# csxmli2016/MARCONet

Hardware: NVIDIA H100
Metric: sr_chars_per_sec (higher is better)
Workload: dtype f32

## Files before the change

marconet_b200/csrc/conv_small.cu:

```cuda
#include "conv_common.cuh"
#include "mn_common.cuh"

namespace {

constexpr int PH = 8, PW = 32, CCH = 16;
constexpr int PIX_PITCH = CCH + 4;

template <int COUT>
__global__ void __launch_bounds__(PH * PW) conv3x3_small_cout_kernel(const ConvGeom g) {
    mn_pdl_prologue();
    __shared__ __align__(16) float halo[(PH + 2) * (PW + 2) * PIX_PITCH];
    __shared__ __align__(16) float wsm[9 * CCH * 4];
    const int tx = threadIdx.x % PW, ty = threadIdx.x / PW;
    const int tiles_w = (g.W + PW - 1) / PW, tiles_h = (g.H + PH - 1) / PH;
    int b = blockIdx.x;
    const int twi = b % tiles_w; b /= tiles_w;
    const int thi = b % tiles_h;
    const int n = b / tiles_h;
    const int ox0 = twi * PW, oy0 = thi * PH;
    const float* xn = g.x + (size_t)n * g.H * g.W * g.x_cs;
    float acc[4] = {0.f, 0.f, 0.f, 0.f};
    for (int c0 = 0; c0 < g.Cin; c0 += CCH) {
        __syncthreads();
        for (int i = threadIdx.x; i < (PH + 2) * (PW + 2) * (CCH / 4); i += PH * PW) {
            const int q = i % (CCH / 4), pix = i / (CCH / 4);
            const int hx = pix % (PW + 2), hy = pix / (PW + 2);
            const int iy = oy0 + hy - 1, ix = ox0 + hx - 1;
            float4 v = make_float4(0.f, 0.f, 0.f, 0.f);
            if ((unsigned)iy < (unsigned)g.H && (unsigned)ix < (unsigned)g.W)
                v = __ldg(reinterpret_cast<const float4*>(xn + ((size_t)iy * g.W + ix) * g.x_cs + c0 + q * 4));
            *reinterpret_cast<float4*>(&halo[pix * PIX_PITCH + q * 4]) = v;
        }
        for (int i = threadIdx.x; i < 9 * CCH * 4; i += PH * PW) {
            const int o = i & 3, c = (i >> 2) % CCH, tap = i / (4 * CCH);
            wsm[i] = o < COUT ? __ldg(g.w + ((size_t)tap * g.Cin + c0 + c) * g.Cout + o) : 0.f;
        }
        __syncthreads();
#pragma unroll
        for (int ky = 0; ky < 3; ++ky)
#pragma unroll
            for (int kx = 0; kx < 3; ++kx) {
                const float* hp = &halo[((ty + ky) * (PW + 2) + tx + kx) * PIX_PITCH];
                const float* wp = &wsm[(ky * 3 + kx) * CCH * 4];
#pragma unroll
                for (int q = 0; q < CCH / 4; ++q) {
                    const float4 a = *reinterpret_cast<const float4*>(hp + q * 4);
                    const float av[4] = {a.x, a.y, a.z, a.w};
#pragma unroll
                    for (int j = 0; j < 4; ++j) {
                        const float4 wv = *reinterpret_cast<const float4*>(wp + (q * 4 + j) * 4);
                        acc[0] = fmaf(av[j], wv.x, acc[0]);
                        if (COUT > 1) acc[1] = fmaf(av[j], wv.y, acc[1]);
                        if (COUT > 2) acc[2] = fmaf(av[j], wv.z, acc[2]);
                        if (COUT > 3) acc[3] = fmaf(av[j], wv.w, acc[3]);
                    }
                }
            }
    }
    const int oy = oy0 + ty, ox = ox0 + tx;
    if (oy < g.H && ox < g.W) {
        const int m = (n * g.H + oy) * g.W + ox;
        conv_epilogue4(g, m, 0, acc);
    }
}

}

bool mn_conv_small_supported(const ConvGeom& g) {
    return g.KH == 3 && g.KW == 3 && g.sh == 1 && g.sw == 1 && g.ph == 1 && g.pw == 1 && g.Cout <= 4 && g.Cin % 16 == 0 &&
           g.x_cs % 4 == 0 && (reinterpret_cast<uintptr_t>(g.x) & 15) == 0;
}

int mn_conv_small_launch(const ConvGeom& g, cudaStream_t st) {
    const int blocks = g.N * ((g.H + PH - 1) / PH) * ((g.W + PW - 1) / PW);
    switch (g.Cout) {
        case 1: MN_CUDA_CHECK((mn_launch(conv3x3_small_cout_kernel<1>, dim3(blocks), dim3(PH * PW), 0, st, g))); break;
        case 2: MN_CUDA_CHECK((mn_launch(conv3x3_small_cout_kernel<2>, dim3(blocks), dim3(PH * PW), 0, st, g))); break;
        case 3: MN_CUDA_CHECK((mn_launch(conv3x3_small_cout_kernel<3>, dim3(blocks), dim3(PH * PW), 0, st, g))); break;
        default: MN_CUDA_CHECK((mn_launch(conv3x3_small_cout_kernel<4>, dim3(blocks), dim3(PH * PW), 0, st, g))); break;
    }
    MN_LAUNCH_CHECK();
    return MN_OK;
}
```

marconet_b200/csrc/conv_tc2.cu:

```cuda
#include <cuda.h>
#include <cuda_bf16.h>
#include <cuda_fp16.h>

#include "conv_common.cuh"
#include "mn_common.cuh"
#include "tc_ptx.cuh"

namespace {
using namespace tcptx;

constexpr int KB = 64;
constexpr int NUM_THREADS2 = 512;
constexpr int REG_SPLIT = 88, REG_PROD = 24, REG_CONS = 200;
static_assert(REG_SPLIT + REG_PROD + 2 * REG_CONS <= 4 * 128, "register budget");
constexpr int MAX_HS = 3;
constexpr int MAX_BSTAGES = 4;
__host__ __device__ constexpr int b_half(int nt) { return nt * 128; }
__host__ __device__ constexpr int b_stage(int nt) { return 2 * b_half(nt); }
constexpr int STG_PITCH = 72;
constexpr int STG_BYTES = 128 * STG_PITCH * 4;
constexpr int SMEM_LIMIT = 232448;

template <int A> struct ActTag { static constexpr int value = A; };

struct GnAcc {
    float p = 0.f, s = 0.f, q = 0.f;
    int c = 0;
    __device__ __forceinline__ void add(const float4 w) {
        if (c == 0) p = w.x;
        const float d0 = w.x - p, d1 = w.y - p, d2 = w.z - p, d3 = w.w - p;
        s += (d0 + d1) + (d2 + d3);
        q = fmaf(d0, d0, fmaf(d1, d1, fmaf(d2, d2, fmaf(d3, d3, q))));
        c += 4;
    }
    __device__ __forceinline__ void sums(double& sum, double& sq) const {
        const double pd = p, cd = c;
        sum = cd * pd + s;
        sq = (double)q + 2.0 * pd * s + cd * pd * pd;
    }
};

template <bool GN, int MODE, int NT>
__global__ void __launch_bounds__(NUM_THREADS2, 1)
conv_tc2_kernel(const __grid_constant__ CUtensorMap tmA, const __grid_constant__ CUtensorMap tmBhi,
                const __grid_constant__ CUtensorMap tmBlo, const ConvGeom g, const Tc2Geom t) {
    constexpr int B_HALF = b_half(NT), B_STAGE = b_stage(NT);
    extern __shared__ uint8_t smem_raw[];
    uint8_t* smem = smem_raw + ((1024u - (smem_u32(smem_raw) & 1023u)) & 1023u);
    const uint32_t smem_base = smem_u32(smem);
    const int HS = t.hstages;
    const uint32_t off_b = HS * t.halo_stage_bytes;
    const uint32_t off_stg = off_b + t.bstages * B_STAGE;
    const uint32_t off_rowm = off_stg + STG_BYTES;
    const uint32_t off_bars = off_rowm + 1024;
    float* stg = reinterpret_cast<float*>(smem + off_stg);
    int* rowm = reinterpret_cast<int*>(smem + off_rowm);
    uint64_t* bars = reinterpret_cast<uint64_t*>(smem + off_bars);
    constexpr int I_HF = 0, I_HE = MAX_HS, I_SD = 2 * MAX_HS, I_BF = 3 * MAX_HS, I_BE = I_BF + MAX_BSTAGES;
    auto bar = [&](int i) { return smem_u32(bars + i); };

    const int warp = threadIdx.x >> 5, lane = threadIdx.x & 31;
    const int cs = t.cs;
    const uint32_t crank = cs > 1 ? cluster_ctarank() : 0u;
    const uint16_t cmask = (uint16_t)((1u << cs) - 1u);
    const int num_clusters = gridDim.x / cs;
    auto first_work = [&]() { return (int)(blockIdx.x / cs); };
    const int total_work = t.m_groups * t.n_tiles * t.ksplit;
    const int BS = t.bstages;
    const int units = t.per_tap ? t.cbps * t.taps : t.cbps;
    const int unit_taps = t.per_tap ? 1 : t.taps;
    auto work_ks = [&](int work) { return work % t.ksplit; };
    auto work_nt = [&](int work) { return (work / t.ksplit) % t.n_tiles; };
    auto work_mg = [&](int work) { return work / (t.ksplit * t.n_tiles); };

    if (threadIdx.x == 0) {
        asm volatile("prefetch.tensormap [%0];" ::"l"(&tmA) : "memory");
        asm volatile("prefetch.tensormap [%0];" ::"l"(&tmBhi) : "memory");
        asm volatile("prefetch.tensormap [%0];" ::"l"(&tmBlo) : "memory");
        for (int s = 0; s < MAX_HS; ++s) { mbar_init(bar(I_HF + s), 1); mbar_init(bar(I_HE + s), 2); mbar_init(bar(I_SD + s), 128); }
        for (int s = 0; s < MAX_BSTAGES; ++s) { mbar_init(bar(I_BF + s), 1); mbar_init(bar(I_BE + s), 2 * cs); }
        fence_barrier_init();
    }
    __syncthreads();
    if (cs > 1) cluster_sync_all();
    asm volatile("griddepcontrol.wait;" ::: "memory");
    asm volatile("griddepcontrol.launch_dependents;" ::: "memory");

    auto tile_origin = [&](int work, int& n0, int& oy0, int& ox0) {
        int m_tile = work_mg(work) * cs + (int)crank;
        if (m_tile >= t.m_tiles) { n0 = g.N + 1024; oy0 = 0; ox0 = 0; return; }
        const int tw_i = m_tile % t.tiles_w; m_tile /= t.tiles_w;
        const int th_i = m_tile % t.tiles_h; m_tile /= t.tiles_h;
        n0 = m_tile * t.TN; oy0 = th_i * t.TH; ox0 = tw_i * t.TW;
    };

    if (warp >= 4 && warp < 8) {
        setmaxnreg_dec<REG_PROD>();
        if (warp == 4) {
            uint32_t s = 0, ph = 0;
            const int rows = NT / cs;
            const uint32_t dst0 = smem_base + off_b + crank * rows * 128;
            for (int work = first_work(); work < total_work; work += num_clusters) {
                const int row0 = work_nt(work) * NT + (int)crank * rows;
                const int cb0 = work_ks(work) * t.cbps;
                for (int cb = cb0; cb < cb0 + t.cbps; ++cb) {
                    for (int tap = 0; tap < t.taps; ++tap) {
                        mbar_wait(bar(I_BE + s), ph ^ 1);
                        if (elect_one_sync()) {
                            const uint32_t dst = dst0 + s * B_STAGE;
                            mbar_expect_tx(bar(I_BF + s), B_STAGE);
                            if (cs > 1) {
                                tma_load_3d_mc(&tmBhi, bar(I_BF + s), dst, cb * KB, row0, tap, cmask);
                                tma_load_3d_mc(&tmBlo, bar(I_BF + s), dst + B_HALF, cb * KB, row0, tap, cmask);
                            } else {
                                tma_load_3d(&tmBhi, bar(I_BF + s), dst, cb * KB, row0, tap);
                                tma_load_3d(&tmBlo, bar(I_BF + s), dst + B_HALF, cb * KB, row0, tap);
                            }
                        }
                        __syncwarp();
                        if (++s == (uint32_t)BS) { s = 0; ph ^= 1; }
                    }
                }
            }
        } else if (warp == 5) {
            uint32_t hs = 0, ph = 0;
            for (int work = first_work(); work < total_work; work += num_clusters) {
                int n0, oy0, ox0;
                tile_origin(work, n0, oy0, ox0);
                const int cb0 = work_ks(work) * t.cbps;
                for (int u = 0; u < units; ++u) {
                    const int cb = cb0 + (t.per_tap ? u / t.taps : u);
                    const int tap = t.per_tap ? u % t.taps : 0;
                    const int ky = tap / t.KW, kx = tap - ky * t.KW;
                    mbar_wait(bar(I_HE + hs), ph ^ 1);
                    if (elect_one_sync()) {
                        mbar_expect_tx(bar(I_HF + hs), 2u * t.halo_rows * 128u);
                        const uint32_t dst = smem_base + hs * t.halo_stage_bytes;
                        tma_load_4d(&tmA, bar(I_HF + hs), dst, cb * KB, ox0 + kx - t.pw, oy0 + ky - t.ph, n0);
                        tma_load_4d(&tmA, bar(I_HF + hs), dst + t.box_bytes, cb * KB + 32, ox0 + kx - t.pw, oy0 + ky - t.ph, n0);
                    }
                    __syncwarp();
                    if (++hs == (uint32_t)HS) { hs = 0; ph ^= 1; }
                }
            }
        }
    } else if (warp < 4) {
        setmaxnreg_dec<REG_SPLIT>();
        const int sidx = threadIdx.x;
        const bool bf = t.prec == MN_PREC_BF16X3_TC;
        const uint32_t mask = bf ? 0xFFFF0000u : 0xFFFFE000u;
        const float xs = g.x_scale;
        float amax = 0.f;
        uint32_t hs = 0, hph = 0;
        const int G = g.Cin >> 5;
        const int qs = sidx & 3, rs0 = sidx >> 2;
        const int rows_up = (t.halo_rows + 31) & ~31;
        for (int work = first_work(); work < total_work; work += num_clusters) {
            int hn0 = 0, hoy0 = 0, hox0 = 0, gvw = 0x7fffffff;
            if (GN) {
                tile_origin(work, hn0, hoy0, hox0);
                if (g.valid_w && hn0 < g.N) gvw = g.valid_w[hn0];
            }
            const int cb0 = work_ks(work) * t.cbps;
            for (int u = 0; u < units; ++u) {
                const int cb = cb0 + (t.per_tap ? u / t.taps : u);
                float gm0 = 0.f, gm1 = 0.f, ga[16], gb[16];
                if (GN) {
#pragma unroll
                    for (int e = 0; e < 16; ++e) { ga[e] = 0.f; gb[e] = 0.f; }
                    if (hn0 < g.N) {
                        const float2 mr0 = g.gn_mr[(size_t)hn0 * G + cb * 2], mr1 = g.gn_mr[(size_t)hn0 * G + cb * 2 + 1];
                        gm0 = mr0.x; gm1 = mr1.x;
#pragma unroll
                        for (int hlf = 0; hlf < 2; ++hlf)
#pragma unroll
                            for (int f = 0; f < 2; ++f) {
                                const int c0 = cb * KB + hlf * 32 + qs * 8 + f * 4;
                                const float4 gg = ldg4(g.gn_gamma + c0), be = ldg4(g.gn_beta + c0);
                                const float rs = hlf ? mr1.y : mr0.y;
                                ga[hlf * 8 + f * 4 + 0] = rs * gg.x; ga[hlf * 8 + f * 4 + 1] = rs * gg.y;
                                ga[hlf * 8 + f * 4 + 2] = rs * gg.z; ga[hlf * 8 + f * 4 + 3] = rs * gg.w;
                                gb[hlf * 8 + f * 4 + 0] = be.x; gb[hlf * 8 + f * 4 + 1] = be.y; gb[hlf * 8 + f * 4 + 2] = be.z; gb[hlf * 8 + f * 4 + 3] = be.w;
                            }
                    }
                }
                mbar_wait(bar(I_HF + hs), hph);
                uint8_t* halo = smem + hs * t.halo_stage_bytes;
                if constexpr (!GN) {
                    auto load8 = [&](const uint8_t* src, int sw, float4 (&v)[8]) {
#pragma unroll
                        for (int j = 0; j < 8; ++j) v[j] = *reinterpret_cast<const float4*>(src + ((j ^ sw) << 4));
                    };
                    auto split16 = [&](float4 (&vv)[8], uint32_t (&hi)[16], uint32_t (&lo)[16]) {
#pragma unroll
                        for (int j = 0; j < 8; ++j) {
                            float4 v = vv[j];
                            v.x *= xs; v.y *= xs; v.z *= xs; v.w *= xs;
                            amax = fmaxf(fmaxf(amax, fabsf(v.x)), fmaxf(fabsf(v.y), fmaxf(fabsf(v.z), fabsf(v.w))));
                            const float h0 = __uint_as_float(__float_as_uint(v.x) & mask), h1 = __uint_as_float(__float_as_uint(v.y) & mask);
                            const float h2 = __uint_as_float(__float_as_uint(v.z) & mask), h3 = __uint_as_float(__float_as_uint(v.w) & mask);
                            if (bf) {
                                hi[2 * j] = pack_bf16(h0, h1); hi[2 * j + 1] = pack_bf16(h2, h3);
                                lo[2 * j] = pack_bf16(v.x - h0, v.y - h1); lo[2 * j + 1] = pack_bf16(v.z - h2, v.w - h3);
                            } else {
                                hi[2 * j] = pack_f16(h0, h1); hi[2 * j + 1] = pack_f16(h2, h3);
                                lo[2 * j] = pack_f16(v.x - h0, v.y - h1); lo[2 * j + 1] = pack_f16(v.z - h2, v.w - h3);
                            }
                        }
                    };
                    auto store4 = [&](uint8_t* dst, int sw, int jj0, const uint32_t (&w)[16]) {
#pragma unroll
                        for (int jj = 0; jj < 4; ++jj)
                            *reinterpret_cast<uint4*>(dst + (((jj0 + jj) ^ sw) << 4)) = make_uint4(w[4 * jj], w[4 * jj + 1], w[4 * jj + 2], w[4 * jj + 3]);
                    };
                    for (int rho = sidx; rho < t.halo_rows; rho += 128) {
                        uint8_t* row0 = halo + rho * 128;
                        uint8_t* row1 = row0 + t.box_bytes;
                        const int sw = rho & 7;
                        float4 v[8];
                        uint32_t hi[16], lo[16];
                        load8(row0, sw, v);
                        split16(v, hi, lo);
                        store4(row0, sw, 0, hi);
                        load8(row1, sw, v);
                        store4(row1, sw, 0, lo);
                        split16(v, hi, lo);
                        store4(row0, sw, 4, hi);
                        store4(row1, sw, 4, lo);
                    }
                } else
                for (int rho = rs0; rho < rows_up; rho += 32) {
                    const bool live = rho < t.halo_rows;
                    uint8_t* row0 = halo + rho * 128;
                    uint8_t* row1 = row0 + t.box_bytes;
                    const int sw = rho & 7;
                    const uint32_t o0 = (uint32_t)((2 * qs) ^ sw) << 4, o1 = (uint32_t)((2 * qs + 1) ^ sw) << 4;
                    float4 v[4];
#pragma unroll
                    for (int k = 0; k < 4; ++k) v[k] = make_float4(0.f, 0.f, 0.f, 0.f);
                    if (live) {
                        v[0] = *reinterpret_cast<const float4*>(row0 + o0); v[1] = *reinterpret_cast<const float4*>(row0 + o1);
                        v[2] = *reinterpret_cast<const float4*>(row1 + o0); v[3] = *reinterpret_cast<const float4*>(row1 + o1);
                    }
                    const int hy = rho / t.HWd, hx = rho - hy * t.HWd;
                    const int y = hoy0 - t.ph + hy, x = hox0 - t.pw + hx;
                    const bool inside = hn0 < g.N && (unsigned)y < (unsigned)g.H && (unsigned)x < (unsigned)g.W && x < gvw;
                    uint32_t hw[8], lw[8];
#pragma unroll
                    for (int k = 0; k < 4; ++k) {
                        float tt[4] = {v[k].x, v[k].y, v[k].z, v[k].w};
                        const float mean = (k >> 1) ? gm1 : gm0;
#pragma unroll
                        for (int e = 0; e < 4; ++e) {
                            float uu = fmaf(tt[e] - mean, ga[k * 4 + e], gb[k * 4 + e]);
                            if (g.gn_swish) uu = __fdividef(uu, 1.f + __expf(-uu));
                            tt[e] = inside ? uu * xs : 0.f;
                        }
                        amax = fmaxf(fmaxf(amax, fabsf(tt[0])), fmaxf(fabsf(tt[1]), fmaxf(fabsf(tt[2]), fabsf(tt[3]))));
                        const float h0 = __uint_as_float(__float_as_uint(tt[0]) & mask), h1 = __uint_as_float(__float_as_uint(tt[1]) & mask);
                        const float h2 = __uint_as_float(__float_as_uint(tt[2]) & mask), h3 = __uint_as_float(__float_as_uint(tt[3]) & mask);
                        if (bf) {
                            hw[2 * k] = pack_bf16(h0, h1); hw[2 * k + 1] = pack_bf16(h2, h3);
                            lw[2 * k] = pack_bf16(tt[0] - h0, tt[1] - h1); lw[2 * k + 1] = pack_bf16(tt[2] - h2, tt[3] - h3);
                        } else {
                            hw[2 * k] = pack_f16(h0, h1); hw[2 * k + 1] = pack_f16(h2, h3);
                            lw[2 * k] = pack_f16(tt[0] - h0, tt[1] - h1); lw[2 * k + 1] = pack_f16(tt[2] - h2, tt[3] - h3);
                        }
                    }
                    __syncwarp();
                    if (live) {
                        const uint32_t ca = (uint32_t)(qs ^ sw) << 4, cb2 = (uint32_t)((4 + qs) ^ sw) << 4;
                        const uint4 ha = make_uint4(hw[0], hw[1], hw[2], hw[3]), hb = make_uint4(hw[4], hw[5], hw[6], hw[7]);
                        const uint4 la = make_uint4(lw[0], lw[1], lw[2], lw[3]), lb = make_uint4(lw[4], lw[5], lw[6], lw[7]);
                        const bool odd = (rho & 1) != 0;
                        const uint32_t c1 = odd ? cb2 : ca, c2 = odd ? ca : cb2;
                        const uint4 h1 = odd ? hb : ha, h2 = odd ? ha : hb, l1 = odd ? lb : la, l2 = odd ? la : lb;
                        *reinterpret_cast<uint4*>(row0 + c1) = h1; *reinterpret_cast<uint4*>(row1 + c1) = l1;
                        *reinterpret_cast<uint4*>(row0 + c2) = h2; *reinterpret_cast<uint4*>(row1 + c2) = l2;
                    }
                }
                asm volatile("fence.proxy.async.shared::cta;" ::: "memory");
                mbar_arrive(bar(I_SD + hs));
                if (++hs == (uint32_t)HS) { hs = 0; hph ^= 1; }
            }
        }
        conv_range_report(g, __float_as_uint(amax), t.prec == MN_PREC_F16X3_TC || t.prec == MN_PREC_F16X1_TC);
    } else {
        setmaxnreg_inc<REG_CONS>();
        const int wg = (warp - 8) >> 2, wq = warp & 3;
        const int wtid = threadIdx.x - 256 - wg * 128;
        constexpr bool bf = MODE == 1, three = MODE != 2;
        const int r = wg * 64 + wq * 16 + (lane & 15);
        const int tn = r / (t.TH * t.TW);
        const int rem = r - tn * (t.TH * t.TW);
        const int th = rem / t.TW, tw = rem - th * t.TW;
        const int rho0 = tn < t.TN ? (tn * t.HHt + th) * t.HWd + tw : 0;
        const uint32_t kchunk = (uint32_t)(lane >> 4);
        const uint64_t desc0 = make_b_desc(smem_base + off_b);
        const float wscale = (t.wscale ? *t.wscale : 1.f) / g.x_scale;
        const float dfix = 1.f + 1.5e-8f * (float)(t.taps * t.cbps * (KB / 16));
        float* wstg = stg + wg * 64 * STG_PITCH;
        auto release_b = [&](uint32_t s) {
            if (cs > 1) { if (lane == 0 && wq < cs) mbar_arrive_cluster(mapa_u32(bar(I_BE + s), (uint32_t)wq)); }
            else if (wtid == 0) mbar_arrive(bar(I_BE + s));
        };
        auto release_a = [&](uint32_t s) { if (wtid == 0) mbar_arrive(bar(I_HE + s)); };
        constexpr int ND = NT / 2;
        uint32_t hs = 0, hph = 0, bs = 0, bph = 0;
        for (int work = first_work(); work < total_work; work += num_clusters) {
            float d[ND], dc[ND];
#pragma unroll
            for (int i = 0; i < ND; ++i) { d[i] = 0.f; dc[i] = 0.f; }
            auto fence_acc = [&]() {
#pragma unroll
                for (int i = 0; i < ND; ++i) { wg_fence_operand(d[i]); if (three) wg_fence_operand(dc[i]); }
            };
            int kb = 0;
            for (int u = 0; u < units; ++u) {
                mbar_wait(bar(I_SD + hs), hph);
                const uint32_t abase = smem_base + hs * t.halo_stage_bytes;
                int ky = 0, kx = 0;
                for (int tap = 0; tap < unit_taps; ++tap, ++kb) {
                    const int rho = rho0 + ky * t.HWd + kx;
                    if (++kx == t.KW) { kx = 0; ++ky; }
                    const uint32_t arow = abase + rho * 128;
                    const uint32_t sw = (uint32_t)(rho & 7);
                    uint32_t ah[4][4], al[4][4];
#pragma unroll
                    for (int j = 0; j < 4; ++j) {
                        const uint32_t off = ((2u * j + kchunk) ^ sw) << 4;
                        ldsm_x4(arow + off, ah[j]);
                        if (three) ldsm_x4(arow + t.box_bytes + off, al[j]);
                    }
                    mbar_wait(bar(I_BF + bs), bph);
                    const uint64_t dh0 = desc0 + (uint64_t)((bs * B_STAGE) >> 4);
                    const uint64_t dl0 = dh0 + (uint64_t)(B_HALF >> 4);
                    fence_acc();
                    wg_fence();
#pragma unroll
                    for (int j = 0; j < 4; ++j) {
                        const uint32_t acc = (kb | j) != 0;
                        wgmma_k16_rs<NT, bf>(d, ah[j], dh0 + 2 * j, acc);
                        if (three) { wgmma_k16_rs<NT, bf>(dc, ah[j], dl0 + 2 * j, acc); wgmma_k16_rs<NT, bf>(dc, al[j], dh0 + 2 * j, 1); }
                    }
                    wg_commit();
                    wg_wait<0>();
                    fence_acc();
                    release_b(bs);
                    if (++bs == (uint32_t)BS) { bs = 0; bph ^= 1; }
                }
                release_a(hs);
                if (++hs == (uint32_t)HS) { hs = 0; hph ^= 1; }
            }

#pragma unroll
            for (int i = 0; i < ND; ++i) d[i] = three ? fmaf(d[i], dfix, dc[i]) * wscale : d[i] * wscale;
            const int nt_i = work_nt(work);
            const int ks = work_ks(work);
            int n0, oy0, ox0;
            tile_origin(work, n0, oy0, ox0);
#pragma unroll 1
            for (int h = 0; h < NT / 64; ++h) {
                named_bar_sync(1 + wg, 128);
                if (h == 0 && wtid < 64) {
                    const int rr = wg * 64 + wtid;
                    const int tn2 = rr / (t.TH * t.TW), rem2 = rr - tn2 * (t.TH * t.TW);
                    const int th2 = rem2 / t.TW, tw2 = rem2 - th2 * t.TW;
                    const int n = n0 + tn2, oy = oy0 + th2, ox = ox0 + tw2;
                    const bool ok = tn2 < t.TN && n < g.N && oy < g.OH && ox < g.OW;
                    rowm[rr] = ok ? (n * g.OH + oy) * g.OW + ox : -1;
                    rowm[128 + rr] = ok ? (n | ((g.valid_w && ox >= g.valid_w[n]) ? (1 << 30) : 0)) : 0;
                }
                {
                    const int row = wq * 16 + (lane >> 2), col = 2 * (lane & 3);
#pragma unroll
                    for (int i = 0; i < 8; ++i) {
                        const int i1 = ND - 32 + 4 * i;
                        const float v0 = h ? d[i1] : d[4 * i], v1 = h ? d[i1 + 1] : d[4 * i + 1];
                        const float v2 = h ? d[i1 + 2] : d[4 * i + 2], v3 = h ? d[i1 + 3] : d[4 * i + 3];
                        *reinterpret_cast<float2*>(wstg + row * STG_PITCH + 8 * i + col) = make_float2(v0, v1);
                        *reinterpret_cast<float2*>(wstg + (row + 8) * STG_PITCH + 8 * i + col) = make_float2(v2, v3);
                    }
                }
                named_bar_sync(1 + wg, 128);
                {
                    const int col = (lane & 15) * 4;
                    const int o = nt_i * NT + h * 64 + col;
                    const int rbase = wg * 64 + wq * 16 + (lane >> 4);
                    if (t.ksplit > 1) {
#pragma unroll 4
                        for (int i = 0; i < 8; ++i) {
                            const int row = rbase + 2 * i;
                            const int m = rowm[row];
                            if (m >= 0)
                                *reinterpret_cast<float4*>(g.ws + ((size_t)ks * g.M + m) * g.Cout + o) =
                                    *reinterpret_cast<const float4*>(stg + row * STG_PITCH + col);
                        }
                    } else {
                        const float4 bias4 = g.bias ? ldg4(g.bias + o) : make_float4(0.f, 0.f, 0.f, 0.f);
                        const bool one_n = t.TN == 1;
                        float4 os4 = make_float4(1.f, 1.f, 1.f, 1.f), y2s4 = os4;
                        float* y2base = g.y2;
                        if (one_n && n0 < g.N) {
                            if (g.out_scale) os4 = ldg4(g.out_scale + (size_t)n0 * g.os_stride + o);
                            if (g.y2 && g.y2_scale) y2s4 = ldg4(g.y2_scale + (size_t)n0 * g.y2s_stride + o);
                            if (g.y2_ptrs) y2base = g.y2_ptrs[n0] - (size_t)n0 * g.OH * g.OW * g.y2_cs;
                        }
                        GnAcc ga;
                        const bool dense_tile = one_n && n0 < g.N && t.TH * t.TW == 128;
                        const int tws = __ffs(t.TW) - 1;
                        const int m00 = (n0 * g.OH + oy0) * g.OW + ox0;
                        const int vwn = (dense_tile && g.valid_w) ? g.valid_w[n0] : 0x7fffffff;
                        auto rows_dense = [&](auto tag) {
                            constexpr int ACT = decltype(tag)::value;
#pragma unroll 4
                            for (int i = 0; i < 8; ++i) {
                                const int row = rbase + 2 * i;
                                const int th3 = row >> tws, tw3 = row & (t.TW - 1);
                                const int m = m00 + th3 * g.OW + tw3;
                                const float4 uv = *reinterpret_cast<const float4*>(stg + row * STG_PITCH + col);
                                const bool masked = ox0 + tw3 >= vwn;
                                const float4 w4 = conv_epilogue_row4<ACT>(g, m, n0, masked, o, uv, bias4, true, os4, true, y2s4, y2base);
                                if (g.gn_stats_out && !masked) ga.add(w4);
                            }
                        };
                        auto rows = [&](auto tag) {
                            constexpr int ACT = decltype(tag)::value;
                            if (dense_tile) { rows_dense(tag); return; }
                            if (one_n && n0 >= g.N) return;
#pragma unroll 4
                            for (int i = 0; i < 8; ++i) {
                                const int row = rbase + 2 * i;
                                const int m = rowm[row];
                                if (m >= 0) {
                                    const int nn = rowm[128 + row];
                                    const float4 uv = *reinterpret_cast<const float4*>(stg + row * STG_PITCH + col);
                                    const bool masked = (nn >> 30) != 0;
                                    const float4 w4 = conv_epilogue_row4<ACT>(g, m, nn & 0x3FFFFFFF, masked, o, uv, bias4, one_n, os4, one_n, y2s4, y2base);
                                    if (g.gn_stats_out && !masked) ga.add(w4);
                                }
                            }
                        };
                        switch (g.act) {
                            case MN_ACT_NONE: rows(ActTag<MN_ACT_NONE>{}); break;
                            case MN_ACT_RELU: rows(ActTag<MN_ACT_RELU>{}); break;
                            case MN_ACT_LRELU02: rows(ActTag<MN_ACT_LRELU02>{}); break;
                            default: rows(ActTag<-1>{}); break;
                        }
                        if (g.gn_stats_out) {
                            double gs, gq;
                            ga.sums(gs, gq);
#pragma unroll
                            for (int sh = 1; sh <= 4; sh <<= 1) { gs += __shfl_xor_sync(0xffffffffu, gs, sh); gq += __shfl_xor_sync(0xffffffffu, gq, sh); }
                            gs += __shfl_xor_sync(0xffffffffu, gs, 16); gq += __shfl_xor_sync(0xffffffffu, gq, 16);
                            if ((lane & 23) == 0 && n0 < g.N) {
                                double* dst = g.gn_stats_out + ((size_t)n0 * (g.Cout >> 5) + (o >> 5)) * 2;
                                atomicAdd(dst, gs);
                                atomicAdd(dst + 1, gq);
                            }
                        }
                    }
                }
            }
        }
    }
    __syncthreads();
    if (cs > 1) cluster_sync_all();
}

typedef CUresult (*PFN_encodeTiled)(CUtensorMap*, CUtensorMapDataType, cuuint32_t, void*, const cuuint64_t*, const cuuint64_t*,
                                    const cuuint32_t*, const cuuint32_t*, CUtensorMapInterleave, CUtensorMapSwizzle,
                                    CUtensorMapL2promotion, CUtensorMapFloatOOBfill);
PFN_encodeTiled get_encode2() {
    static PFN_encodeTiled fn = nullptr;
    if (!fn) {
        void* p = nullptr;
        cudaDriverEntryPointQueryResult q;
        if (cudaGetDriverEntryPoint("cuTensorMapEncodeTiled", &p, cudaEnableDefault, &q) == cudaSuccess && q == cudaDriverEntryPointSuccess)
            fn = reinterpret_cast<PFN_encodeTiled>(p);
    }
    return fn;
}

bool is_pow2(int v) { return v > 0 && (v & (v - 1)) == 0; }

bool plan_common(const ConvGeom& g, Tc2Plan& p) {
    auto fail = [&](const char* w) { p.ok = false; p.why = w; return false; };
    if (g.sh != 1 || g.sw != 1) return fail("stride != 1");
    const bool k3 = g.KH == 3 && g.KW == 3 && g.ph == 1 && g.pw == 1, k1 = g.KH == 1 && g.KW == 1 && g.ph == 0 && g.pw == 0;
    if (!k3 && !k1) return fail("only 3x3/pad1 and 1x1/pad0");
    if (g.Cin % KB != 0) return fail("Cin % 64 != 0");
    if (g.Cout % 64 != 0) return fail("Cout % 64 != 0");
    if (g.x_cs % 4 != 0 || (reinterpret_cast<uintptr_t>(g.x) & 15)) return fail("x alignment");
    auto al16 = [](const void* q) { return (reinterpret_cast<uintptr_t>(q) & 15) == 0; };
    if ((g.y && (g.y_cs % 4 || !al16(g.y))) || (g.y2 && (g.y2_cs % 4 || !al16(g.y2))) || (g.residual && (g.res_cs % 4 || !al16(g.residual))) ||
        (g.out_scale && (g.os_stride % 4 || !al16(g.out_scale))) || (g.y2_scale && (g.y2s_stride % 4 || !al16(g.y2_scale))) ||
        (g.bias && !al16(g.bias)))
        return fail("epilogue operands must be 16-byte aligned with channel strides that are multiples of 4");
    p.t.KW = g.KW;
    p.t.cblocks = g.Cin / KB; p.t.taps = g.KH * g.KW;
    return true;
}

void plan_nt(const ConvGeom& g, Tc2Plan& p, bool allow_ksplit, int nt) {
    Tc2Geom& t = p.t;
    t.nt = nt;
    t.n_tiles = g.Cout / nt;
    t.ksplit = 1;
    if (allow_ksplit) {
        const int items = t.m_groups * t.n_tiles, slots = mn_num_sms() / t.cs;
        while (t.ksplit * 2 * items <= slots && t.cblocks % (t.ksplit * 2) == 0 && t.ksplit < 8) t.ksplit *= 2;
        while (t.ksplit > 1 && (int64_t)t.ksplit * g.M * g.Cout * 4 > g.ws_bytes) t.ksplit >>= 1;
        if (t.ksplit > 1 && (!g.ws || g.gn_mr || (g.Cout & 3) || g.y2_ptrs || g.gn_stats_out)) t.ksplit = 1;
    }
    t.cbps = t.cblocks / t.ksplit;
    const int other = STG_BYTES + 1024 + 256 + 1024;
    const int units = t.per_tap ? t.cbps * t.taps : t.cbps;
    t.hstages = 2;
    if (3 * t.halo_stage_bytes + other + 3 * b_stage(nt) <= SMEM_LIMIT && (t.per_tap || (units <= 4 && units >= 2))) t.hstages = 3;
    const int fixed = t.hstages * t.halo_stage_bytes + other;
    int bs = (SMEM_LIMIT - fixed) / b_stage(nt);
    if (bs > MAX_BSTAGES) bs = MAX_BSTAGES;
    t.bstages = bs;
    p.smem = fixed + bs * b_stage(nt);
}

int64_t plan_cost(const Tc2Geom& t) {
    const int clusters = mn_num_sms() / t.cs;
    const int64_t waves = (t.m_groups * t.n_tiles * t.ksplit + clusters - 1) / clusters;
    return waves * (t.nt / 64) * t.cbps;
}

bool plan_finish(const ConvGeom& g, Tc2Plan& p, bool allow_ksplit) {
    Tc2Geom& t = p.t;
    t.box_bytes = (t.halo_rows * 128 + 1023) & ~1023;
    t.halo_stage_bytes = 2 * t.box_bytes;
    t.m_tiles = t.tiles_w * t.tiles_h * t.tiles_n;
    t.cs = t.m_tiles >= 2 ? 2 : 1;
    t.m_groups = (t.m_tiles + t.cs - 1) / t.cs;
    plan_nt(g, p, allow_ksplit, 64);
    if (g.Cout % 128 == 0) {
        Tc2Plan wide = p;
        plan_nt(g, wide, allow_ksplit, 128);
        const int64_t cw = plan_cost(wide.t), cn = plan_cost(p.t);
        if (wide.t.bstages >= 3 && (cw < cn || (cw == cn && wide.t.ksplit <= p.t.ksplit))) p = wide;
    }
    if (t.bstages < 2) { p.ok = false; p.why = "not enough shared memory for 2 weight stages"; return false; }
    p.ok = true;
    return true;
}

Tc2Plan plan_tc2(ConvGeom& g) {
    Tc2Plan p{};
    auto fail = [&](const char* w) { p.ok = false; p.why = w; return p; };
    if (!plan_common(g, p)) return p;
    Tc2Geom& t = p.t;
    t.per_tap = 0;
    t.TH = g.H < 8 ? g.H : 8;
    if (!is_pow2(t.TH) || g.H % t.TH) return fail("H must be a multiple of 8 (or a power of two below 8)");
    const int maxw = 128 / t.TH;
    t.TW = g.W < maxw ? g.W : maxw;
    if (!is_pow2(t.TW) || g.W % t.TW) return fail("W must be a multiple of 128/TH (or a power of two below it)");
    t.TN = 128 / (t.TH * t.TW);
    t.ph = g.ph; t.pw = g.pw;
    t.HHt = t.TH + 2 * g.ph; t.HWd = t.TW + 2 * g.pw;
    while (t.TN > 1 && t.TN * t.HHt * t.HWd > 208) t.TN >>= 1;
    t.halo_rows = t.TN * t.HHt * t.HWd;
    if (t.halo_rows > 208) return fail("halo tile too large for shared memory");
    if (g.y2_ptrs && t.TN != 1) return fail("per-sample output pointers need samples of at least one whole pixel tile (OH*OW >= 128)");
    if (t.TN != 1) { g.gn_mr = nullptr; g.gn_stats_out = nullptr; }
    if (t.HWd > 256 || t.HHt > 256 || t.TN > 256) return fail("TMA box dim");
    t.tiles_w = g.W / t.TW; t.tiles_h = g.H / t.TH; t.tiles_n = (g.N + t.TN - 1) / t.TN;
    plan_finish(g, p, true);
    return p;
}

Tc2Plan plan_tc1(const ConvGeom& g) {
    Tc2Plan p{};
    auto fail = [&](const char* w) { p.ok = false; p.why = w; return p; };
    if (!plan_common(g, p)) return p;
    Tc2Geom& t = p.t;
    t.per_tap = 1;
    int TW, TH, TN;
    if (g.W >= 128) { if (g.W % 128) return fail("W % 128"); TW = 128; TH = 1; TN = 1; }
    else {
        if (128 % g.W) return fail("W does not divide 128");
        TW = g.W;
        const int rows = 128 / TW;
        if (g.H >= rows) { if (g.H % rows) return fail("H % tile rows"); TH = rows; TN = 1; }
        else { if (rows % g.H) return fail("H does not divide tile rows"); TH = g.H; TN = rows / g.H; }
    }
    t.TW = TW; t.TH = TH; t.TN = TN;
    t.HWd = TW; t.HHt = TH; t.ph = g.ph; t.pw = g.pw;
    t.halo_rows = 128;
    t.tiles_w = g.W / TW; t.tiles_h = g.H / TH; t.tiles_n = (g.N + TN - 1) / TN;
    plan_finish(g, p, false);
    return p;
}

template <bool GN, int MODE, int NT>
int launch_tc2(const CUtensorMap& ma, const CUtensorMap& mbh, const CUtensorMap& mbl, const ConvGeom& g, const Tc2Plan& p, cudaStream_t st) {
    static unsigned long long smem_done = 0;
    MN_CUDA_CHECK(mn_ensure_dyn_smem(conv_tc2_kernel<GN, MODE, NT>, SMEM_LIMIT, &smem_done));
    const Tc2Geom& t = p.t;
    cudaLaunchConfig_t cfg{};
    cfg.gridDim = dim3(mn_conv_tc_ctas(t), 1, 1);
    cfg.blockDim = dim3(NUM_THREADS2, 1, 1);
    cfg.dynamicSmemBytes = p.smem;
    cfg.stream = st;
    cudaLaunchAttribute attr[2];
    attr[0].id = cudaLaunchAttributeClusterDimension;
    attr[0].val.clusterDim.x = t.cs; attr[0].val.clusterDim.y = 1; attr[0].val.clusterDim.z = 1;
    attr[1].id = cudaLaunchAttributeProgrammaticStreamSerialization;
    attr[1].val.programmaticStreamSerializationAllowed = 1;
    cfg.attrs = attr; cfg.numAttrs = mn_pdl_enabled() ? 2 : 1;
    MN_CUDA_CHECK(cudaLaunchKernelEx(&cfg, conv_tc2_kernel<GN, MODE, NT>, ma, mbh, mbl, g, t));
    return MN_OK;
}

template <bool GN, int MODE>
int launch_tc2_nt(const CUtensorMap& ma, const CUtensorMap& mbh, const CUtensorMap& mbl, const ConvGeom& g, const Tc2Plan& p, cudaStream_t st) {
    return p.t.nt == 128 ? launch_tc2<GN, MODE, 128>(ma, mbh, mbl, g, p, st) : launch_tc2<GN, MODE, 64>(ma, mbh, mbl, g, p, st);
}

}

int mn_conv_tc_ctas(const Tc2Geom& t) {
    const int total_work = t.m_groups * t.n_tiles * t.ksplit;
    int sms = mn_num_sms();
    if (mn_max_ctas() > 0 && mn_max_ctas() < sms) sms = mn_max_ctas();
    int clusters = sms / t.cs;
    if (clusters < 1) clusters = 1;
    if (clusters > total_work) clusters = total_work;
    return clusters * t.cs;
}

Tc2Plan mn_conv_tc_plan(ConvGeom& g) {
    const Tc2Plan halo = plan_tc2(g);
    if (halo.ok) return halo;
    if (g.y2_ptrs) {
        mn_set_error("mn_conv2d_nhwc: per-sample output pointers (y2_ptrs) exist only in the tensor-core halo tiling, which does not run this shape (%s)", halo.why);
        return halo;
    }
    g.gn_mr = nullptr; g.gn_stats_out = nullptr;
    const Tc2Plan per_tap = plan_tc1(g);
    if (!per_tap.ok)
        mn_set_error("tensor-core path unsupported: halo tiling: %s; per-tap tiling: %s", halo.why, per_tap.why);
    return per_tap;
}

int mn_conv_tc_launch(const ConvGeom& g, Tc2Plan& p, const void* w_hi, const void* w_lo, const float* w_scale, int prec, cudaStream_t st) {
    if (!w_hi || !w_lo || !w_scale) { mn_set_error("mn_conv2d_nhwc: tensor-core precision needs packed w_tc_hi/w_tc_lo/w_tc_scale"); return MN_ERR_INVALID; }
    PFN_encodeTiled enc = get_encode2();
    if (!enc) { mn_set_error("cuTensorMapEncodeTiled not available from the driver"); return MN_ERR_CUDA; }
    CUtensorMap ma, mbh, mbl;
    Tc2Geom& t = p.t;
    {
        cuuint64_t dims[4] = {(cuuint64_t)g.Cin, (cuuint64_t)g.W, (cuuint64_t)g.H, (cuuint64_t)g.N};
        cuuint64_t strides[3] = {(cuuint64_t)g.x_cs * 4, (cuuint64_t)g.W * g.x_cs * 4, (cuuint64_t)g.H * g.W * g.x_cs * 4};
        cuuint32_t box[4] = {32, (cuuint32_t)t.HWd, (cuuint32_t)t.HHt, (cuuint32_t)t.TN};
        cuuint32_t es[4] = {1, 1, 1, 1};
        CUresult r = enc(&ma, CU_TENSOR_MAP_DATA_TYPE_FLOAT32, 4, const_cast<float*>(g.x), dims, strides, box, es,
                         CU_TENSOR_MAP_INTERLEAVE_NONE, CU_TENSOR_MAP_SWIZZLE_128B, CU_TENSOR_MAP_L2_PROMOTION_L2_128B,
                         CU_TENSOR_MAP_FLOAT_OOB_FILL_NONE);
        if (r != CUDA_SUCCESS) { mn_set_error("cuTensorMapEncodeTiled(A) failed: %d", (int)r); return MN_ERR_CUDA; }
    }
    const CUtensorMapDataType dt = (prec == MN_PREC_BF16X3_TC) ? CU_TENSOR_MAP_DATA_TYPE_BFLOAT16 : CU_TENSOR_MAP_DATA_TYPE_FLOAT16;
    for (int which = 0; which < 2; ++which) {
        cuuint64_t dims[3] = {(cuuint64_t)g.Cin, (cuuint64_t)g.Cout, (cuuint64_t)(g.KH * g.KW)};
        cuuint64_t strides[2] = {(cuuint64_t)g.Cin * 2, (cuuint64_t)g.Cin * g.Cout * 2};
        cuuint32_t box[3] = {64, (cuuint32_t)(t.nt / t.cs), 1};
        cuuint32_t es[3] = {1, 1, 1};
        CUresult r = enc(which ? &mbl : &mbh, dt, 3, const_cast<void*>(which ? w_lo : w_hi), dims, strides, box, es,
                         CU_TENSOR_MAP_INTERLEAVE_NONE, CU_TENSOR_MAP_SWIZZLE_128B, CU_TENSOR_MAP_L2_PROMOTION_L2_256B,
                         CU_TENSOR_MAP_FLOAT_OOB_FILL_NONE);
        if (r != CUDA_SUCCESS) { mn_set_error("cuTensorMapEncodeTiled(B) failed: %d", (int)r); return MN_ERR_CUDA; }
    }
    t.wscale = w_scale + 1;
    t.prec = prec;
    int rc;
    if (prec == MN_PREC_BF16X3_TC) rc = g.gn_mr ? launch_tc2_nt<true, 1>(ma, mbh, mbl, g, p, st) : launch_tc2_nt<false, 1>(ma, mbh, mbl, g, p, st);
    else if (prec == MN_PREC_F16X1_TC) rc = g.gn_mr ? launch_tc2_nt<true, 2>(ma, mbh, mbl, g, p, st) : launch_tc2_nt<false, 2>(ma, mbh, mbl, g, p, st);
    else rc = g.gn_mr ? launch_tc2_nt<true, 0>(ma, mbh, mbl, g, p, st) : launch_tc2_nt<false, 0>(ma, mbh, mbl, g, p, st);
    if (rc != MN_OK || t.ksplit == 1) return rc;
    ConvGeom gr = g;
    gr.splits = t.ksplit;
    return mn_conv_splitk_reduce_launch(gr, st);
}
```

Baseline: 1355.

## Register-block small-Cout 3x3 conv over four rows and specialize GN-swish convert path

After: 1375, median of 6. 1.01x the previous value.

```diff
diff --git a/marconet_b200/csrc/conv_small.cu b/marconet_b200/csrc/conv_small.cu
--- a/marconet_b200/csrc/conv_small.cu
+++ b/marconet_b200/csrc/conv_small.cu
@@ -3,15 +3,21 @@
 
 namespace {
 
-constexpr int PH = 8, PW = 32, CCH = 16;
+constexpr int PH = 16, PW = 32, CCH = 16;
+constexpr int RPT = 4;
+constexpr int THREADS = PW * (PH / RPT);
 constexpr int PIX_PITCH = CCH + 4;
+constexpr int HALO_FLOATS = (PH + 2) * (PW + 2) * PIX_PITCH;
+constexpr int W_FLOATS = 9 * CCH * 4;
+constexpr int SMEM_BYTES = (HALO_FLOATS + W_FLOATS) * 4;
 
 template <int COUT>
-__global__ void __launch_bounds__(PH * PW) conv3x3_small_cout_kernel(const ConvGeom g) {
+__global__ void __launch_bounds__(THREADS, 4) conv3x3_small_cout_kernel(const ConvGeom g) {
     mn_pdl_prologue();
-    __shared__ __align__(16) float halo[(PH + 2) * (PW + 2) * PIX_PITCH];
-    __shared__ __align__(16) float wsm[9 * CCH * 4];
-    const int tx = threadIdx.x % PW, ty = threadIdx.x / PW;
+    extern __shared__ __align__(16) float smem_small[];
+    float* halo = smem_small;
+    float* wsm = smem_small + HALO_FLOATS;
+    const int tx = threadIdx.x % PW, ty0 = (threadIdx.x / PW) * RPT;
     const int tiles_w = (g.W + PW - 1) / PW, tiles_h = (g.H + PH - 1) / PH;
     int b = blockIdx.x;
     const int twi = b % tiles_w; b /= tiles_w;
@@ -19,10 +25,12 @@
     const int n = b / tiles_h;
     const int ox0 = twi * PW, oy0 = thi * PH;
     const float* xn = g.x + (size_t)n * g.H * g.W * g.x_cs;
-    float acc[4] = {0.f, 0.f, 0.f, 0.f};
+    float acc[RPT][4];
+#pragma unroll
+    for (int r = 0; r < RPT; ++r) acc[r][0] = acc[r][1] = acc[r][2] = acc[r][3] = 0.f;
     for (int c0 = 0; c0 < g.Cin; c0 += CCH) {
         __syncthreads();
-        for (int i = threadIdx.x; i < (PH + 2) * (PW + 2) * (CCH / 4); i += PH * PW) {
+        for (int i = threadIdx.x; i < (PH + 2) * (PW + 2) * (CCH / 4); i += THREADS) {
             const int q = i % (CCH / 4), pix = i / (CCH / 4);
             const int hx = pix % (PW + 2), hy = pix / (PW + 2);
             const int iy = oy0 + hy - 1, ix = ox0 + hx - 1;
@@ -31,36 +39,44 @@
                 v = __ldg(reinterpret_cast<const float4*>(xn + ((size_t)iy * g.W + ix) * g.x_cs + c0 + q * 4));
             *reinterpret_cast<float4*>(&halo[pix * PIX_PITCH + q * 4]) = v;
         }
-        for (int i = threadIdx.x; i < 9 * CCH * 4; i += PH * PW) {
+        for (int i = threadIdx.x; i < W_FLOATS; i += THREADS) {
             const int o = i & 3, c = (i >> 2) % CCH, tap = i / (4 * CCH);
             wsm[i] = o < COUT ? __ldg(g.w + ((size_t)tap * g.Cin + c0 + c) * g.Cout + o) : 0.f;
         }
         __syncthreads();
-#pragma unroll
+#pragma unroll 1
         for (int ky = 0; ky < 3; ++ky)
 #pragma unroll
             for (int kx = 0; kx < 3; ++kx) {
-                const float* hp = &halo[((ty + ky) * (PW + 2) + tx + kx) * PIX_PITCH];
+                const float* hp = &halo[((ty0 + ky) * (PW + 2) + tx + kx) * PIX_PITCH];
                 const float* wp = &wsm[(ky * 3 + kx) * CCH * 4];
 #pragma unroll
                 for (int q = 0; q < CCH / 4; ++q) {
-                    const float4 a = *reinterpret_cast<const float4*>(hp + q * 4);
-                    const float av[4] = {a.x, a.y, a.z, a.w};
+                    float av[RPT][4];
+#pragma unroll
+                    for (int r = 0; r < RPT; ++r) {
+                        const float4 a = *reinterpret_cast<const float4*>(hp + r * (PW + 2) * PIX_PITCH + q * 4);
+                        av[r][0] = a.x; av[r][1] = a.y; av[r][2] = a.z; av[r][3] = a.w;
+                    }
 #pragma unroll
                     for (int j = 0; j < 4; ++j) {
                         const float4 wv = *reinterpret_cast<const float4*>(wp + (q * 4 + j) * 4);
-                        acc[0] = fmaf(av[j], wv.x, acc[0]);
-                        if (COUT > 1) acc[1] = fmaf(av[j], wv.y, acc[1]);
-                        if (COUT > 2) acc[2] = fmaf(av[j], wv.z, acc[2]);
-                        if (COUT > 3) acc[3] = fmaf(av[j], wv.w, acc[3]);
+#pragma unroll
+                        for (int r = 0; r < RPT; ++r) {
+                            acc[r][0] = fmaf(av[r][j], wv.x, acc[r][0]);
+                            if (COUT > 1) acc[r][1] = fmaf(av[r][j], wv.y, acc[r][1]);
+                            if (COUT > 2) acc[r][2] = fmaf(av[r][j], wv.z, acc[r][2]);
+                            if (COUT > 3) acc[r][3] = fmaf(av[r][j], wv.w, acc[r][3]);
+                        }
                     }
                 }
             }
     }
-    const int oy = oy0 + ty, ox = ox0 + tx;
-    if (oy < g.H && ox < g.W) {
-        const int m = (n * g.H + oy) * g.W + ox;
-        conv_epilogue4(g, m, 0, acc);
+    const int ox = ox0 + tx;
+#pragma unroll
+    for (int r = 0; r < RPT; ++r) {
+        const int oy = oy0 + ty0 + r;
+        if (oy < g.H && ox < g.W) conv_epilogue4(g, (n * g.H + oy) * g.W + ox, 0, acc[r]);
     }
 }
 
@@ -71,13 +87,21 @@
            g.x_cs % 4 == 0 && (reinterpret_cast<uintptr_t>(g.x) & 15) == 0;
 }
 
+template <int COUT>
+cudaError_t launch_small(const ConvGeom& g, int blocks, cudaStream_t st) {
+    static unsigned long long smem_done = 0;
+    const cudaError_t e = mn_ensure_dyn_smem(conv3x3_small_cout_kernel<COUT>, SMEM_BYTES, &smem_done);
+    if (e != cudaSuccess) return e;
+    return mn_launch(conv3x3_small_cout_kernel<COUT>, dim3(blocks), dim3(THREADS), SMEM_BYTES, st, g);
+}
+
 int mn_conv_small_launch(const ConvGeom& g, cudaStream_t st) {
     const int blocks = g.N * ((g.H + PH - 1) / PH) * ((g.W + PW - 1) / PW);
     switch (g.Cout) {
-        case 1: MN_CUDA_CHECK((mn_launch(conv3x3_small_cout_kernel<1>, dim3(blocks), dim3(PH * PW), 0, st, g))); break;
-        case 2: MN_CUDA_CHECK((mn_launch(conv3x3_small_cout_kernel<2>, dim3(blocks), dim3(PH * PW), 0, st, g))); break;
-        case 3: MN_CUDA_CHECK((mn_launch(conv3x3_small_cout_kernel<3>, dim3(blocks), dim3(PH * PW), 0, st, g))); break;
-        default: MN_CUDA_CHECK((mn_launch(conv3x3_small_cout_kernel<4>, dim3(blocks), dim3(PH * PW), 0, st, g))); break;
+        case 1: MN_CUDA_CHECK(launch_small<1>(g, blocks, st)); break;
+        case 2: MN_CUDA_CHECK(launch_small<2>(g, blocks, st)); break;
+        case 3: MN_CUDA_CHECK(launch_small<3>(g, blocks, st)); break;
+        default: MN_CUDA_CHECK(launch_small<4>(g, blocks, st)); break;
     }
     MN_LAUNCH_CHECK();
     return MN_OK;
diff --git a/marconet_b200/csrc/conv_tc2.cu b/marconet_b200/csrc/conv_tc2.cu
--- a/marconet_b200/csrc/conv_tc2.cu
+++ b/marconet_b200/csrc/conv_tc2.cu
@@ -246,27 +246,32 @@
                     const int y = hoy0 - t.ph + hy, x = hox0 - t.pw + hx;
                     const bool inside = hn0 < g.N && (unsigned)y < (unsigned)g.H && (unsigned)x < (unsigned)g.W && x < gvw;
                     uint32_t hw[8], lw[8];
-#pragma unroll
-                    for (int k = 0; k < 4; ++k) {
-                        float tt[4] = {v[k].x, v[k].y, v[k].z, v[k].w};
-                        const float mean = (k >> 1) ? gm1 : gm0;
-#pragma unroll
-                        for (int e = 0; e < 4; ++e) {
-                            float uu = fmaf(tt[e] - mean, ga[k * 4 + e], gb[k * 4 + e]);
-                            if (g.gn_swish) uu = __fdividef(uu, 1.f + __expf(-uu));
-                            tt[e] = inside ? uu * xs : 0.f;
+                    auto convert = [&](auto swish) {
+#pragma unroll
+                        for (int k = 0; k < 4; ++k) {
+                            float tt[4] = {v[k].x, v[k].y, v[k].z, v[k].w};
+                            const float mean = (k >> 1) ? gm1 : gm0;
+#pragma unroll
+                            for (int e = 0; e < 4; ++e) {
+                                float uu = fmaf(tt[e] - mean, ga[k * 4 + e], gb[k * 4 + e]);
+                                if constexpr (decltype(swish)::value != 0)
+                                    uu = __fdividef(uu, 1.f + __expf(-uu));
+                                tt[e] = inside ? uu * xs : 0.f;
+                            }
+                            amax = fmaxf(fmaxf(amax, fabsf(tt[0])), fmaxf(fabsf(tt[1]), fmaxf(fabsf(tt[2]), fabsf(tt[3]))));
+                            const float h0 = __uint_as_float(__float_as_uint(tt[0]) & mask), h1 = __uint_as_float(__float_as_uint(tt[1]) & mask);
+                            const float h2 = __uint_as_float(__float_as_uint(tt[2]) & mask), h3 = __uint_as_float(__float_as_uint(tt[3]) & mask);
+                            if constexpr (MODE == 1) {
+                                hw[2 * k] = pack_bf16(h0, h1); hw[2 * k + 1] = pack_bf16(h2, h3);
+                                lw[2 * k] = pack_bf16(tt[0] - h0, tt[1] - h1); lw[2 * k + 1] = pack_bf16(tt[2] - h2, tt[3] - h3);
+                            } else {
+                                hw[2 * k] = pack_f16(h0, h1); hw[2 * k + 1] = pack_f16(h2, h3);
+                                lw[2 * k] = pack_f16(tt[0] - h0, tt[1] - h1); lw[2 * k + 1] = pack_f16(tt[2] - h2, tt[3] - h3);
+                            }
                         }
-                        amax = fmaxf(fmaxf(amax, fabsf(tt[0])), fmaxf(fabsf(tt[1]), fmaxf(fabsf(tt[2]), fabsf(tt[3]))));
-                        const float h0 = __uint_as_float(__float_as_uint(tt[0]) & mask), h1 = __uint_as_float(__float_as_uint(tt[1]) & mask);
-                        const float h2 = __uint_as_float(__float_as_uint(tt[2]) & mask), h3 = __uint_as_float(__float_as_uint(tt[3]) & mask);
-                        if (bf) {
-                            hw[2 * k] = pack_bf16(h0, h1); hw[2 * k + 1] = pack_bf16(h2, h3);
-                            lw[2 * k] = pack_bf16(tt[0] - h0, tt[1] - h1); lw[2 * k + 1] = pack_bf16(tt[2] - h2, tt[3] - h3);
-                        } else {
-                            hw[2 * k] = pack_f16(h0, h1); hw[2 * k + 1] = pack_f16(h2, h3);
-                            lw[2 * k] = pack_f16(tt[0] - h0, tt[1] - h1); lw[2 * k + 1] = pack_f16(tt[2] - h2, tt[3] - h3);
-                        }
-                    }
+                    };
+                    if (g.gn_swish) convert(ActTag<1>{});
+                    else convert(ActTag<0>{});
                     __syncwarp();
                     if (live) {
                         const uint32_t ca = (uint32_t)(qs ^ sw) << 4, cb2 = (uint32_t)((4 + qs) ^ sw) << 4;
```
